# BoxLib-Codes/VARDEN

Measured on AMD Instinct MI355X. Metric: cells*steps/sec on advance_timestep, higher is better.
Workload: dtype f64; 1 GPU; 3D 256x256x256 single-level variable-density bubble, 1 box(es) of 256^3, MAC+HG projection each step (BASELINE.json configs[1]); parallelism=single GPU, cells=16777216

## Files before the change

### varden_amd/csrc/mg_cc.hip

```cpp
#include "vdn_dev.h"
#include "mg_stop.h"
#include "krylov_wg.h"
#include "krylov_grid.h"
#include <chrono>
#include <tuple>
#include <algorithm>

struct CLev {
  int n[3]; int PX, PY; long sz;
  double hi2[3];
  double *phi, *rh, *res, *b[3];
  double *alpha;
  const double *rho;
  int fold[3][2];
  double cmu;
};
DEVI long cidx(const CLev &L, int i, int j, int k) { return (long)(i + 16) + (long)L.PX * ((long)(j + 1) + (long)L.PY * (long)(k + 1)); }

DEVI double beta_of(double ra, double rb, bool at_face, int e) {
  double v = 2.0 / (ra + rb);
  if (at_face) { if (e == VDN_BC_NEU) v = 0.0; else if (e == VDN_BC_DIR) v = 2.0 * v; }
  return v;
}
template <bool RHO = false> DEVI void cc_apply(const CLev &L, long c, double &Ap, double &diag, int i = 0, int j = 0, int k = 0) {
  const long sy = L.PX, sz = (long)L.PX * L.PY;
  const double p0 = L.phi[c];
// ... 652 lines not shown
  DEVI void fill_point(double *v, int t) const { CLev Lv = L; Lv.phi = v; cc_periodic_point(Lv, per, t); }
  KRY_HD long size() const { return L.sz; }
  DEVI const double *rhs() const { return L.rh; }
  DEVI double *x() const { return L.phi; }
  KRY_HD bool singular() const { return sing != 0; }
};
using CcKrylov = CcKrylovT<false>;
using CcKrylovRef = CcKrylovT<true>;
template <bool KRYLOV> __global__ void __launch_bounds__(1024) kk_cc_tailcycle(CcTailArgs T, KrylovTail<KRYLOV> Q) {
  #pragma unroll
  for (int l = 0; l < CC_TAIL_MAX - 1; l++)
    if (l < T.nlev - 1) { wg_cc_gsrb(T.L[l], T.nu1, T.per); wg_cc_down(T.L[l], T.L[l + 1], T.per); }
  #pragma unroll
  for (int l = 0; l < CC_TAIL_MAX; l++)
    if (l == T.nlev - 1) {
      if constexpr (KRYLOV) wg_krylov_any(Q.method, CcKrylovRef{ T.L[l], T.per, Q.singular }, Q.K);
      else wg_cc_gsrb(T.L[l], T.nbot, T.per);
    }
  #pragma unroll
  for (int l = CC_TAIL_MAX - 2; l >= 0; l--)
    if (l < T.nlev - 1) { wg_cc_up(T.L[l], T.L[l + 1]); wg_cc_gsrb(T.L[l], T.nu2, T.per); }
}

constexpr int LT = 8;
constexpr int LW = LT + 8;
struct LdsCell { double b[6], rh, a0; };
template <bool ALPHA> DEVI void lds_load_cell(const CLev &L, long c, LdsCell &q) {
  const long sy = L.PX, sz = (long)L.PX * L.PY;
  q.b[0] = L.b[0][c]; q.b[1] = L.b[0][c + 1]; q.b[2] = L.b[1][c]; q.b[3] = L.b[1][c + sy]; q.b[4] = L.b[2][c]; q.b[5] = L.b[2][c + sz];
  q.rh = L.rh[c]; q.a0 = ALPHA ? L.alpha[c] : 0.0;
}
template <bool ALPHA, int SX, int SP> DEVI void lds_pass(const CLev &L, double *s, const LdsCell (&q)[4], const bool (&inside)[4], int at, int x, int y, int z0, int par0, int color, int reach) {
  const bool xy_ok = x >= 4 - reach && x < 4 + LT + reach && y >= 4 - reach && y < 4 + LT + reach;
  #pragma unroll
  for (int m = 0; m < 4; m++) {
    const int z = z0 + m;
    if (!(xy_ok && inside[m] && z >= 4 - reach && z < 4 + LT + reach && ((par0 + m + color) & 1) == 0)) continue;
    const int a = at + m * SP;
    const double p[7] = { s[a], s[a - 1], s[a + 1], s[a - SX], s[a + SX], s[a - SP], s[a + SP] };
    double Ap, diag; cc_apply_vals(L, p, q[m].b, q[m].a0, ALPHA, Ap, diag);
    if (diag != 0.0) s[a] = p[0] + (q[m].rh - Ap) / diag;
  }
}
template <bool ALPHA> __global__ void __launch_bounds__(1024) kk_cc_lds_down(CLev L, CLev C) {
  constexpr int SX = LW + 2, SP = SX * SX;
  __shared__ double s[SX * SX * SX];
// ... 560 lines not shown
}

static void cc_periodic_t(const CCMG &M, const CLev &L) {
  if (!(M.per[0] || M.per[1] || M.per[2])) return;
  int m = std::max(L.n[0], std::max(L.n[1], L.n[2]));
  hipLaunchKernelGGL(kk_cc_periodic, g3(m, m, 6, BLK), BLK, 0, ctx().stream, L, M.per[0], M.per[1], M.per[2]);
}
static void cc_gsrb_t(const CCMG &M, const CLev &L, int nsweeps) {
  if ((long)L.n[0] * L.n[1] * L.n[2] <= SMALL_LEVEL_CELLS) {
    hipLaunchKernelGGL(kk_cc_bottom, dim3(1), dim3(1024), 0, ctx().stream, L, nsweeps, M.per[0], M.per[1], M.per[2]);
    return;
  }
  for (int s = 0; s < nsweeps; s++) for (int color = 0; color < 2; color++) {
    cc_periodic_t(M, L);
    launch_gsrb(L, color, ctx().stream);
  }
}
static void cc_bottom_t(const CCMG &M, const CLev &L) {
  if (M.kry.w) { mg_krylov_visit(M.kry, 0, ctx().prm.mg_bottom_solver_eps, M.krylov(L)); return; }
  const int N = std::max(L.n[0], std::max(L.n[1], L.n[2]));
  const int ns = std::max(ctx().prm.mg_nub, N * N);
  hipLaunchKernelGGL(kk_cc_bottom, dim3(1), dim3(1024), 0, ctx().stream, L, ns, M.per[0], M.per[1], M.per[2]);
}
static bool cc_small_end(const CCMG &M, int dl, int tl) {
  if (!sw().mg_tailcycle) return false;
  static const long tail_cells = SMALL_LEVEL_CELLS;
  const vdn_params &P = ctx().prm;
  CcTailArgs T; memset(&T, 0, sizeof T);
  int nl = 0;
  if (dl >= 0) {
    if (!M.tail.empty() && !(ctx().nranks == 1 && M.dlev.back().single_box)) return false;
    for (int m = dl; m < (int)M.dlev.size(); m++) {
      const CDLev &D = M.dlev[m];
      if (!(D.single_box && D.boxes.size() == 1 && !D.boxes[0].L.rho && (long)D.ng[0] * D.ng[1] * D.ng[2] <= tail_cells) || nl == CC_TAIL_MAX) return false;
      T.L[nl++] = D.boxes[0].L;
    }
  }
  for (int m = tl; m < (int)M.tail.size(); m++) {
    const CLev &L = M.tail[m];
    if ((long)L.n[0] * L.n[1] * L.n[2] > tail_cells || nl == CC_TAIL_MAX) return false;
    T.L[nl++] = L;
  }
  if (nl < 2) return false;
  const CLev &B = T.L[nl - 1];
  const int N = std::max(B.n[0], std::max(B.n[1], B.n[2]));
  T.nlev = nl; T.nu1 = P.mg_nu1; T.nu2 = P.mg_nu2; T.nbot = std::max(P.mg_nub, N * N);
  for (int d = 0; d < 3; d++) T.per[d] = M.per[d];
  if (M.kry.w) hipLaunchKernelGGL(kk_cc_tailcycle<true>, dim3(1), dim3(1024), 0, ctx().stream, T, KrylovTailArgs{ mg_krylov_args(M.kry, 0, P.mg_bottom_solver_eps), M.kry.method, M.kry_singular });
  else hipLaunchKernelGGL(kk_cc_tailcycle<false>, dim3(1), dim3(1024), 0, ctx().stream, T, NoKrylovTailArgs{});
  return true;
}
static bool cc_lds_tail_level(const CCMG &M, int l) {
  const vdn_params &P = ctx().prm;
  if (!sw().mg_lds || l + 1 >= (int)M.tail.size() || P.mg_nu1 != 2 || P.mg_nu2 != 2 || M.per[0] || M.per[1] || M.per[2]) return false;
  const CLev &L = M.tail[l], &C = M.tail[l + 1];
  if (L.rho) return false;
  for (int d = 0; d < 3; d++) if (L.n[d] % LT || L.n[d] < 2 * LT || L.n[d] > 64 || C.n[d] * 2 != L.n[d]) return false;
  return true;
}
static void cc_vcycle_t(const CCMG &M, int l) {
  const vdn_params &P = ctx().prm;
  if (cc_small_end(M, -1, l)) return;
  const CLev &L = M.tail[l];
  if (l == (int)M.tail.size() - 1) { cc_bottom_t(M, L); return; }
  const CLev &C = M.tail[l + 1];
  if (cc_lds_tail_level(M, l)) {
    const dim3 g((unsigned)(L.n[0] / LT), (unsigned)(L.n[1] / LT), (unsigned)(L.n[2] / LT));
    if (L.alpha) hipLaunchKernelGGL(kk_cc_lds_down<true>, g, dim3(1024), 0, ctx().stream, L, C);
    else hipLaunchKernelGGL(kk_cc_lds_down<false>, g, dim3(1024), 0, ctx().stream, L, C);
    cc_vcycle_t(M, l + 1);
    if (L.alpha) hipLaunchKernelGGL(kk_cc_lds_up<true>, g, dim3(1024), 0, ctx().stream, L, C);
    else hipLaunchKernelGGL(kk_cc_lds_up<false>, g, dim3(1024), 0, ctx().stream, L, C);
    return;
  }
// ... 699 lines not shown
```

### varden_amd/csrc/mg_nd.hip

```cpp
#include "vdn_dev.h"
#include "mg_stop.h"
#include "krylov_wg.h"
#include "krylov_grid.h"
#include "nd_lds_plan.h"
#include <tuple>
#include <algorithm>

struct NLev {
  int n[3]; int PX, PY; long sz;
  double f[3];
  double *phi, *tmp, *b, *res, *sig;
  int dirlo[3], dirhi[3];
  int per[3];
};
DEVI long nidx(const NLev &L, int i, int j, int k) { return (long)(i + 16) + (long)L.PX * ((long)(j + 1) + (long)L.PY * (long)(k + 1)); }
DEVI bool nd_is_dir(const NLev &L, int i, int j, int k) {
  return (i == 0 && L.dirlo[0]) || (i == L.n[0] && L.dirhi[0]) || (j == 0 && L.dirlo[1]) || (j == L.n[1] && L.dirhi[1]) ||
         (k == 0 && L.dirlo[2]) || (k == L.n[2] && L.dirhi[2]);
}
DEVI bool nd_is_shell(const NLev &L, int i, int j, int k, int hm) {
  return ((hm & 1) && i == 0) || ((hm & 2) && i == L.n[0]) || ((hm & 4) && j == 0) || ((hm & 8) && j == L.n[1]) ||
         ((hm & 16) && k == 0) || ((hm & 32) && k == L.n[2]);
}

struct NdW { double w0, w1, w2, w3, w4, w5, w6, w7; int iso; };
DEVI NdW nd_weights(const double f[3]) {
  const double fx = f[0], fy = f[1], fz = f[2];
  const double F = fx + fy + fz;
  NdW W;
  W.w0 = 4.0 * F;
  W.w1 = -4.0 * fx + 2.0 * fy + 2.0 * fz;
  W.w2 = 2.0 * fx - 4.0 * fy + 2.0 * fz;
  W.w3 = -2.0 * fx - 2.0 * fy + fz;
  W.w4 = 2.0 * fx + 2.0 * fy - 4.0 * fz;
  W.w5 = -2.0 * fx + fy - 2.0 * fz;
  W.w6 = fx - 2.0 * fy - 2.0 * fz;
  W.w7 = -F;
  W.iso = (W.w1 == 0.0 && W.w2 == 0.0 && W.w4 == 0.0);
  return W;
}
DEVI void nd_stencil(const NdW &W, const double p[3][3][3], const double sg[2][2][2], double &Kp, double &diag) {
  double cz[2][2], cy[2][2], cx[2][2];
  #pragma unroll
  for (int b = 0; b < 2; b++)
    #pragma unroll
    for (int a = 0; a < 2; a++) {
      cz[b][a] = sg[0][b][a] + sg[1][b][a];
      cy[b][a] = sg[b][0][a] + sg[b][1][a];
      cx[b][a] = sg[b][a][0] + sg[b][a][1];
    }
  const double S8 = (cz[0][0] + cz[0][1]) + (cz[1][0] + cz[1][1]);
  const double p0 = p[1][1][1];
  #define D(c, b, a) (p[c][b][a] - p0)
  double A7 = sg[0][0][0] * D(0, 0, 0);
  A7 = fma(sg[0][0][1], D(0, 0, 2), A7); A7 = fma(sg[0][1][0], D(0, 2, 0), A7); A7 = fma(sg[0][1][1], D(0, 2, 2), A7);
  A7 = fma(sg[1][0][0], D(2, 0, 0), A7); A7 = fma(sg[1][0][1], D(2, 0, 2), A7); A7 = fma(sg[1][1][0], D(2, 2, 0), A7); A7 = fma(sg[1][1][1], D(2, 2, 2), A7);
  double A3 = cz[0][0] * D(1, 0, 0); A3 = fma(cz[0][1], D(1, 0, 2), A3); A3 = fma(cz[1][0], D(1, 2, 0), A3); A3 = fma(cz[1][1], D(1, 2, 2), A3);
  double A5 = cy[0][0] * D(0, 1, 0); A5 = fma(cy[0][1], D(0, 1, 2), A5); A5 = fma(cy[1][0], D(2, 1, 0), A5); A5 = fma(cy[1][1], D(2, 1, 2), A5);
  double A6 = cx[0][0] * D(0, 0, 1); A6 = fma(cx[0][1], D(0, 2, 1), A6); A6 = fma(cx[1][0], D(2, 0, 1), A6); A6 = fma(cx[1][1], D(2, 2, 1), A6);
  const double dg = W.w0 * S8;
  double acc = W.w3 * A3;
  acc = fma(W.w5, A5, acc); acc = fma(W.w6, A6, acc); acc = fma(W.w7, A7, acc);
  if (!W.iso) {
    double A1 = (cz[0][0] + cz[1][0]) * D(1, 1, 0); A1 = fma(cz[0][1] + cz[1][1], D(1, 1, 2), A1);
    double A2 = (cz[0][0] + cz[0][1]) * D(1, 0, 1); A2 = fma(cz[1][0] + cz[1][1], D(1, 2, 1), A2);
    double A4 = (cy[0][0] + cy[0][1]) * D(0, 1, 1); A4 = fma(cy[1][0] + cy[1][1], D(2, 1, 1), A4);
    acc = fma(W.w1, A1, acc); acc = fma(W.w2, A2, acc); acc = fma(W.w4, A4, acc);
  }
  #undef D
  Kp = acc; diag = dg;
}
DEVI void nd_apply(const NLev &L, const double *__restrict__ phi, int i, int j, int k, double &Kp, double &diag) {
  const NdW W = nd_weights(L.f);
  const long sy = L.PX, sz = (long)L.PX * L.PY;
  const long c0 = nidx(L, i, j, k);
  double p[3][3][3], sg[2][2][2];
  #pragma unroll
  for (int c = 0; c < 3; c++)
    #pragma unroll
    for (int b = 0; b < 3; b++)
      #pragma unroll
      for (int a = 0; a < 3; a++) p[c][b][a] = phi[c0 + (a - 1) + (b - 1) * sy + (c - 1) * sz];
  #pragma unroll
  for (int c = 0; c < 2; c++)
    #pragma unroll
    for (int b = 0; b < 2; b++)
      #pragma unroll
      for (int a = 0; a < 2; a++) sg[c][b][a] = L.sig[c0 + (a - 1) + (b - 1) * sy + (c - 1) * sz];
  nd_stencil(W, p, sg, Kp, diag);
}

#define NODE_IJK(L)                                                    \
  const int i = blockIdx.x * blockDim.x + threadIdx.x;                 \
// ... 389 lines not shown
  const int k = (int)blockIdx.z - 1;
  if (i > L.n[0] || j > L.n[1] || k > L.n[2]) return;
  int q[3] = { i, j, k }, s[3] = { i, j, k }; bool g = false, zero = false;
  #pragma unroll
  for (int d = 0; d < 3; d++) {
    if (q[d] < 0) { g = true; if (L.per[d]) s[d] = q[d] + L.n[d]; else zero = true; }
    else if (q[d] >= L.n[d]) { g = true; if (L.per[d]) s[d] = q[d] - L.n[d]; else zero = true; }
  }
  if (g) a[nidx(L, i, j, k)] = zero ? 0.0 : a[nidx(L, s[0], s[1], s[2])];
}
__global__ void kk_nd_restrict(NLev F, NLev C) {
  NODE_IJK(C)
  if (!in_range) return;
  double s = 0.0;
  if (!nd_is_dir(C, i, j, k)) {
    const long sy = F.PX, sz = (long)F.PX * F.PY;
    const long f0 = nidx(F, 2 * i, 2 * j, 2 * k);
    s = nd_fw27(F.res + f0, sy, sz);
  }
  const long cn = nidx(C, i, j, k);
  C.b[cn] = s * 0.125;
  C.phi[cn] = 0.0;
}
DEVI double nd_interp8(const NLev &C, const double *__restrict__ cp, int I, int J, int K, int oi, int oj, int ok) {
  const long c0 = nidx(C, I, J, K), sy = C.PX, sz = (long)C.PX * C.PY;
  const double v000 = cp[c0], v100 = cp[c0 + 1], v010 = cp[c0 + sy], v110 = cp[c0 + sy + 1];
  const double v001 = cp[c0 + sz], v101 = cp[c0 + sz + 1], v011 = cp[c0 + sz + sy], v111 = cp[c0 + sz + sy + 1];
  double s = 0.0;
  s = s + v000;
  s = oi ? s + v100 : s;
  s = oj ? s + v010 : s;
  s = (oi && oj) ? s + v110 : s;
  s = ok ? s + v001 : s;
  s = (ok && oi) ? s + v101 : s;
  s = (ok && oj) ? s + v011 : s;
  s = (ok && oi && oj) ? s + v111 : s;
  return s * (1.0 / (double)((1 + oi) * (1 + oj) * (1 + ok)));
}
__global__ void __launch_bounds__(256) kk_nd_prolong_m(NLev F, NLev C, int c00, int c01, int c02, int kchunk) {
  const int i = blockIdx.x * 64 + threadIdx.x, j = blockIdx.y * 4 + threadIdx.y;
  const int k0 = (int)blockIdx.z * kchunk, k1 = min(k0 + kchunk - 1, F.n[2]);
  if (i > F.n[0] || j > F.n[1] || k0 > k1) return;
  const int oi = i & 1, oj = j & 1;
  const long sy = C.PX, sz = (long)C.PX * C.PY;
  const double *__restrict__ cp = C.phi;
  long c0 = nidx(C, c00 + (i >> 1), c01 + (j >> 1), c02 + (k0 >> 1));
  double a00 = cp[c0], a10 = cp[c0 + 1], a01 = cp[c0 + sy], a11 = cp[c0 + sy + 1];
  const bool dir_ij = (i == 0 && F.dirlo[0]) || (i == F.n[0] && F.dirhi[0]) || (j == 0 && F.dirlo[1]) || (j == F.n[1] && F.dirhi[1]);
  const double w0 = 1.0 / (double)((1 + oi) * (1 + oj)), w1 = 1.0 / (double)((1 + oi) * (1 + oj) * 2);
  for (int k = k0; k <= k1; k += 2) {
    const double b00 = cp[c0 + sz], b10 = cp[c0 + sz + 1], b01 = cp[c0 + sz + sy], b11 = cp[c0 + sz + sy + 1];
    const long f = nidx(F, i, j, k);
    const double pe = F.phi[f];
    const bool odd_in = k + 1 <= k1;
    const long f2 = f + (long)F.PX * F.PY;
    const double po = odd_in ? F.phi[f2] : 0.0;
    double s = 0.0;
    s = s + a00;
    s = oi ? s + a10 : s;
    s = oj ? s + a01 : s;
// ... 297 lines not shown
  KRY_HD long size() const { return L.sz; }
  DEVI const double *rhs() const { return L.b; }
  DEVI double *x() const { return phi; }
  KRY_HD bool singular() const { return !(L.dirlo[0] || L.dirlo[1] || L.dirlo[2] || L.dirhi[0] || L.dirhi[1] || L.dirhi[2]); }
};
using NdKrylov = NdKrylovT<false>;
using NdKrylovRef = NdKrylovT<true>;
template <bool KRYLOV> __global__ void __launch_bounds__(1024) kk_nd_tailcycle(NdTailArgs T, KrylovTail<KRYLOV> Q) {
  double *ph[ND_TAIL_MAX], *tm[ND_TAIL_MAX];
  #pragma unroll
  for (int l = 0; l < ND_TAIL_MAX; l++) { ph[l] = T.L[l].phi; tm[l] = T.L[l].tmp; }
  #pragma unroll
  for (int l = 0; l < ND_TAIL_MAX - 1; l++)
    if (l < T.nlev - 1) { wg_nd_jacobi(T.L[l], ph[l], tm[l], T.nu1, T.omega, T.om1, T.om2, T.nsp); wg_nd_down(T.L[l], ph[l], T.L[l + 1], ph[l + 1]); }
  #pragma unroll
  for (int l = 0; l < ND_TAIL_MAX; l++)
    if (l == T.nlev - 1) {
      if constexpr (KRYLOV) wg_krylov_any(Q.method, NdKrylovRef{ T.L[l], ph[l] }, Q.K);
      else wg_nd_jacobi(T.L[l], ph[l], tm[l], T.nbot, T.omega);
    }
  #pragma unroll
  for (int l = ND_TAIL_MAX - 2; l >= 0; l--)
    if (l < T.nlev - 1) { wg_nd_up(T.L[l], ph[l], T.L[l + 1], ph[l + 1]); wg_nd_jacobi(T.L[l], ph[l], tm[l], T.nu2, T.omega); }
}

__global__ void kk_nd_load_sigma(NLev L, FV coeffs, int lo0, int lo1, int lo2) {
  const int i = (int)(blockIdx.x * blockDim.x + threadIdx.x) - 1;
  const int j = (int)(blockIdx.y * blockDim.y + threadIdx.y) - 1;
  const int k = (int)blockIdx.z - 1;
  if (i > L.n[0] || j > L.n[1] || k > L.n[2]) return;
  L.sig[nidx(L, i, j, k)] = fv_get(coeffs, lo0 + i, lo1 + j, lo2 + k);
}
DEVI void nd_divu_node(const FV &u, const FV &rh, double fx, double fy, double fz, int i, int j, int k) {
  #define U(a, b, c, m) fv_get(u, i + (a), j + (b), k + (c), m)
  const double dux = (((U(0, 0, 0, 0) + U(0, -1, 0, 0)) + U(0, 0, -1, 0)) + U(0, -1, -1, 0))
                   - (((U(-1, 0, 0, 0) + U(-1, -1, 0, 0)) + U(-1, 0, -1, 0)) + U(-1, -1, -1, 0));
  const double duy = (((U(0, 0, 0, 1) + U(-1, 0, 0, 1)) + U(0, 0, -1, 1)) + U(-1, 0, -1, 1))
                   - (((U(0, -1, 0, 1) + U(-1, -1, 0, 1)) + U(0, -1, -1, 1)) + U(-1, -1, -1, 1));
  const double duz = (((U(0, 0, 0, 2) + U(-1, 0, 0, 2)) + U(0, -1, 0, 2)) + U(-1, -1, 0, 2))
                   - (((U(0, 0, -1, 2) + U(-1, 0, -1, 2)) + U(0, -1, -1, 2)) + U(-1, -1, -1, 2));
  #undef U
  fv_at(rh, i, j, k) = fv_get(rh, i, j, k) + (dux * fx + duy * fy + duz * fz);
}
struct nd_divu_K { FV u; FV rh; double fx; double fy; double fz;
  __device__ void cell(int i, int j, int k) const {
    nd_divu_node(u, rh, fx, fy, fz, i, j, k);
// ... 457 lines not shown
static bool nd_prolong_fusable(const NDMG &M, int l) {
  const NDLev &DL = M.dlev[l];
  if (!(sw().nd_prolong_fused && DL.single_box && DL.boxes.size() == 1 && !DL.halo_A && !DL.halo_B && !(DL.per[0] || DL.per[1] || DL.per[2]))) return false;
  if (l + 1 < (int)M.dlev.size() ? M.dlev[l + 1].boxes.size() != 1 : M.tail.empty()) return false;
  const NBox &B = DL.boxes[0];
  const NLev &L = B.L, &C = l + 1 < (int)M.dlev.size() ? M.dlev[l + 1].boxes[0].L : M.tail[0];
  for (int d = 0; d < 3; d++) if (B.lo[d] != 0 || C.n[d] != L.n[d] / 2) return false;
  return nd_wide_even_level(L);
}
static unsigned g_nd_pro_levels = 0;
unsigned nd_last_prolong_levels() { return g_nd_pro_levels; }
static void nd_prolong_smooth(NDMG &M, int l) {
  const int nu2 = ctx().prm.hg_nu2;
  if (nu2 < 1 || !nd_prolong_fusable(M, l)) { nd_prolong_up(M, l); nd_jacobi_d(M.dlev[l], nu2); return; }
  if (l + 1 < (int)M.dlev.size()) nd_halo_phi(M.dlev[l + 1]); else nd_fill_nodes(M.tail[0], M.tail[0].phi);
  const NLev C = l + 1 < (int)M.dlev.size() ? M.dlev[l + 1].boxes[0].L : M.tail[0];
  M.pro_levels |= 1u << l;
  nd_jacobi_d(M.dlev[l], nu2, false, &C);
}
static int nd_bottom_sweeps_global(const NDLev &DL) {
  const int N = std::max(DL.ng[0], std::max(DL.ng[1], DL.ng[2]));
  return std::max(ctx().prm.hg_nub, 2 * N * N);
}
static bool nd_small_end(NDMG &M, int dl, int tl) {
  if (!sw().mg_tailcycle) return false;
  static const long tail_nodes = SMALL_LEVEL_NODES;
  const vdn_params &P = ctx().prm;
  NdTailArgs T; memset(&T, 0, sizeof T);
  int nl = 0;
  if (dl >= 0) {
    if (!M.tail.empty() && !(ctx().nranks == 1 && M.dlev.back().single_box)) return false;
    for (int m = dl; m < (int)M.dlev.size(); m++) {
      const NDLev &D = M.dlev[m];
      if (!(D.single_box && D.boxes.size() == 1 && (long)(D.ng[0] + 1) * (D.ng[1] + 1) * (D.ng[2] + 1) <= tail_nodes) || nl == ND_TAIL_MAX) return false;
      T.L[nl] = D.boxes[0].L; for (int d = 0; d < 3; d++) T.L[nl].per[d] = D.per[d];
      nl++;
    }
  }
  for (int m = tl; m < (int)M.tail.size(); m++) {
    const NLev &L = M.tail[m];
    if ((long)(L.n[0] + 1) * (L.n[1] + 1) * (L.n[2] + 1) > tail_nodes || nl == ND_TAIL_MAX) return false;
    T.L[nl++] = L;
  }
  if (nl < 2) return false;
  const NLev &B = T.L[nl - 1];
  const int N = std::max(B.n[0], std::max(B.n[1], B.n[2]));
  T.nlev = nl; T.nu1 = P.hg_nu1; T.nu2 = P.hg_nu2; T.nbot = std::max(P.hg_nub, 2 * N * N); T.omega = P.hg_omega; { const NdOm o = nd_om(true, P.hg_nu1); T.om1 = o.om1; T.om2 = o.om2; T.nsp = o.nsp; }
  if (M.kry.w) { hipLaunchKernelGGL(kk_nd_tailcycle<true>, dim3(1), dim3(1024), 0, ctx().stream, T, KrylovTailArgs{ mg_krylov_args(M.kry, 1, P.hg_bottom_solver_eps), M.kry.method, 0 }); T.nbot = 0;  }
  else hipLaunchKernelGGL(kk_nd_tailcycle<false>, dim3(1), dim3(1024), 0, ctx().stream, T, NoKrylovTailArgs{});
  int m = 0;
  if (dl >= 0) for (int q = dl; q < (int)M.dlev.size(); q++, m++) {
    const int sweeps = (m == nl - 1) ? T.nbot : T.nu1 + T.nu2;
    if (sweeps & 1) { NDLev &D = M.dlev[q]; std::swap(D.boxes[0].L.phi, D.boxes[0].L.tmp); D.flip = !D.flip; }
  }
  for (int q = tl; q < (int)M.tail.size(); q++, m++) {
    const int sweeps = (m == nl - 1) ? T.nbot : T.nu1 + T.nu2;
    if (sweeps & 1) std::swap(M.tail[q].phi, M.tail[q].tmp);
  }
  return true;
}
static bool nd_lds_level(const NDMG &M, int l) {
  const vdn_params &P = ctx().prm;
  if (!sw().mg_lds || l < 1 || l + 1 >= (int)M.dlev.size() || ctx().nranks != 1 || P.hg_nu1 != 2 || P.hg_nu2 != 1 || M.per[0] || M.per[1] || M.per[2]) return false;
  const NDLev &D = M.dlev[l], &DC = M.dlev[l + 1];
  if (!(D.single_box && D.boxes.size() == 1 && !D.halo_A && !D.halo_B && !D.halo_res && !(D.per[0] || D.per[1] || D.per[2]) && DC.single_box && DC.boxes.size() == 1)) return false;
  const NBox &B = D.boxes[0];
  for (int d = 0; d < 3; d++) if (!nd_lds_extent_ok(B.L.n[d]) || B.lo[d] != 0 || DC.boxes[0].L.n[d] * 2 != B.L.n[d]) return false;
  return true;
}
static unsigned g_nd_lds_levels = 0;
unsigned nd_last_lds_levels() { return g_nd_lds_levels; }
static void nd_vcycle_d(NDMG &M, int l) {
// ... 1093 lines not shown
```

### varden_amd/csrc/runtime.hip

```cpp
#include "vdn_dev.h"
#include <algorithm>
#include <chrono>
#include <map>
#include <tuple>

static VdnCtx g_ctx;
VdnCtx &ctx() { return g_ctx; }
static thread_local char g_err[1024] = "";

void vdn_set_error(const char *fmt, ...) { va_list ap; va_start(ap, fmt); vsnprintf(g_err, sizeof g_err, fmt, ap); va_end(ap); }
void vdn_fail(const char *fmt, ...) {
  char buf[1024]; va_list ap; va_start(ap, fmt); vsnprintf(buf, sizeof buf, fmt, ap); va_end(ap);
  throw VdnErr(buf);
}

static std::vector<vdn_multifab *> g_temp_mfs;
void arena_reset() {
  dbg_sync(16);
  for (vdn_multifab *m : g_temp_mfs) delete m;
  g_temp_mfs.clear();
  if (sw().arena_poison && g_ctx.arena && g_ctx.arena_peak > 0) HIPCHK(hipMemsetAsync(g_ctx.arena, 0xFF, std::min(g_ctx.arena_peak + (size_t)(64 << 20), g_ctx.arena_bytes), g_ctx.stream));
  g_ctx.arena_off = 0;
  g_ctx.drop_step_caches();
}
// ... 141 lines not shown
extern char **environ;
static void env_warn_unknown() {
  static bool done = false;
  if (done) return;
  done = true;
  for (char **e = environ; e && *e; e++) {
    if (strncmp(*e, "VDN_", 4) != 0 || !strncmp(*e, "VDN_BENCH_", 10) || !strncmp(*e, "VDN_WORKER_", 11)) continue;
    const char *eq = strchr(*e, '=');
    const size_t len = eq ? (size_t)(eq - *e) : strlen(*e);
    bool known = false;
    for (const SwitchInfo &s : switch_table) if (strlen(s.name) == len && !strncmp(s.name, *e, len)) known = true;
    if (!strncmp(*e, "VDN_LIB_FLAVOUR", 15)) continue;
    if (!known) fprintf(stderr, "varden_amd: warning: environment variable %.*s is not a switch of this library (vdn_debug_switches lists them)\n", (int)len, *e);
#ifndef VDN_TESTING_BUILD
    else fprintf(stderr, "varden_amd: note: %.*s is set but this is the release build: launch-form switches are compiled out (libvarden_amd_testing.so reads them)\n", (int)len, *e);
#endif
  }
}
#ifdef VDN_TESTING_BUILD
unsigned nd_last_prolong_levels();
extern "C" unsigned vdn_nd_prolong_fused_levels(void) { return nd_last_prolong_levels(); }
unsigned nd_last_lds_levels();
extern "C" unsigned vdn_nd_lds_levels(void) { return nd_last_lds_levels(); }
#endif
extern "C" const char *vdn_debug_switches(void) {
  static std::string out;
#ifndef VDN_TESTING_BUILD
  if (out.empty()) out = "release build: the switches below are compiled out, every launch form is the default one (libvarden_amd_testing.so reads them)\n";
#endif
  if (out.find(std::string(switch_table[0].name) + " ") == std::string::npos) for (const SwitchInfo &s : switch_table) { const char *v = switch_raw(s); out += s.name; out += v ? std::string(" = ") + v : std::string(" (unset)"); out += ": "; out += s.doc; out += "\n"; }
  return out.c_str();
}

bool g_capturing_now();
__global__ void k_publish(double *host_view, const double *dev, int n, unsigned long long seq) {
  if ((int)threadIdx.x < n) host_view[threadIdx.x] = dev[threadIdx.x];
  __syncthreads();
  if (threadIdx.x == 0) { __threadfence_system(); *reinterpret_cast<volatile unsigned long long *>(host_view + 64) = seq; }
}
const double *read_scalars(const double *dev, int n) {
  VdnCtx &c = g_ctx;
  REQUIRE(n >= 1 && n <= 64, "read_scalars: 1..64 values");
  static unsigned long long seq = 0;
  const bool poll = sw().poll >= 0 ? sw().poll != 0 : c.nranks == 1;
  ++seq;
  dbg_sync(8);
// ... 750 lines not shown
```

Before: 688.1 million cells*steps/s.

## Run small multigrid tail V-cycles entirely in LDS for cell and node solvers

```diff
diff --git a/varden_amd/csrc/mg_cc.hip b/varden_amd/csrc/mg_cc.hip
--- a/varden_amd/csrc/mg_cc.hip
+++ b/varden_amd/csrc/mg_cc.hip
@@ -2,6 +2,7 @@
 #include "mg_stop.h"
 #include "krylov_wg.h"
 #include "krylov_grid.h"
+#include "tail_plan.h"
 #include <chrono>
 #include <tuple>
 #include <algorithm>
@@ -700,6 +701,115 @@
     if (l < T.nlev - 1) { wg_cc_up(T.L[l], T.L[l + 1]); wg_cc_gsrb(T.L[l], T.nu2, T.per); }
 }
 
+struct CcTailLdsArgs { CLev L[TAIL_MAX_LEVELS]; TailPlan P; int nu1, nu2, nbot, per[3]; };
+struct CcOwn {
+  double b[6], a0, rh, diag, res;
+  long gc;
+  int lc, rc, up;
+  int fine;
+  int colour, img;
+  bool ok;
+};
+DEVI void cct_enter(const CcTailLdsArgs &T, int l, CcOwn &o) {
+  const CLev &L = T.L[l]; const TailLevel &P = T.P.L[l];
+  int i, j, k;
+  o.ok = tail_owner(TAIL_CELLS, P.n, threadIdx.x, i, j, k, o.colour);
+  o.gc = cidx(L, i, j, k);
+  o.lc = P.phi + tail_index(P, i, j, k);
+  o.rc = T.P.res + i + P.n[0] * (j + P.n[1] * k);
+  o.up = l + 1 < T.P.nlev ? T.P.L[l + 1].phi + tail_index(T.P.L[l + 1], i >> 1, j >> 1, k >> 1) : 0;
+  o.fine = l > 0 ? T.P.res + 2 * i + T.P.L[l - 1].n[0] * (2 * j + T.P.L[l - 1].n[1] * 2 * k) : 0;
+  o.img = 0;
+  const int q[3] = { i, j, k };
+  for (int d = 0; d < 3; d++) if (T.per[d]) { if (q[d] == 0) o.img |= 1 << (2 * d); if (q[d] == P.n[d] - 1) o.img |= 2 << (2 * d); }
+  const long sy = L.PX, sz = (long)L.PX * L.PY;
+  for (int m = 0; m < 6; m++) o.b[m] = 0.0;
+  o.a0 = 0.0; o.rh = 0.0; o.res = 0.0;
+  if (o.ok) {
+    o.b[0] = L.b[0][o.gc]; o.b[1] = L.b[0][o.gc + 1];
+    o.b[2] = L.b[1][o.gc]; o.b[3] = L.b[1][o.gc + sy];
+    o.b[4] = L.b[2][o.gc]; o.b[5] = L.b[2][o.gc + sz];
+    if (L.alpha) o.a0 = L.alpha[o.gc];
+    if (l == 0) o.rh = L.rh[o.gc];
+  }
+  const double p[7] = { 0.0, 0.0, 0.0, 0.0, 0.0, 0.0, 0.0 };
+  double Ap; cc_apply_vals(L, p, o.b, o.a0, L.alpha != nullptr, Ap, o.diag);
+}
+DEVI double cct_apply(const CLev &L, const TailLevel &P, const double *lds, const CcOwn &o, double &p0) {
+  const int sy = P.e[0], sz = P.e[0] * P.e[1];
+  const double p[7] = { lds[o.lc], lds[o.lc - 1], lds[o.lc + 1], lds[o.lc - sy], lds[o.lc + sy], lds[o.lc - sz], lds[o.lc + sz] };
+  double Ap, diag; cc_apply_vals(L, p, o.b, o.a0, L.alpha != nullptr, Ap, diag);
+  p0 = p[0];
+  return Ap;
+}
+DEVI void cct_put(const TailLevel &P, double *lds, const CcOwn &o, double v) {
+  lds[o.lc] = v;
+  if (o.img) {
+    const int st[3] = { 1, P.e[0], P.e[0] * P.e[1] };
+    #pragma unroll
+    for (int d = 0; d < 3; d++) {
+      if (o.img & (1 << (2 * d))) lds[o.lc + P.n[d] * st[d]] = v;
+      if (o.img & (2 << (2 * d))) lds[o.lc - P.n[d] * st[d]] = v;
+    }
+  }
+}
+DEVI void cct_gsrb(const CLev &L, const TailLevel &P, double *lds, const CcOwn &o, int nsweeps) {
+  for (int s = 0; s < nsweeps; s++) for (int color = 0; color < 2; color++) {
+    if (o.ok && o.colour == color) {
+      double p0; const double Ap = cct_apply(L, P, lds, o, p0);
+      if (o.diag != 0.0) cct_put(P, lds, o, p0 + (o.rh - Ap) / o.diag);
+    }
+    __syncthreads();
+  }
+}
+__global__ void __launch_bounds__(TAIL_THREADS) kk_cc_tailcycle_lds(CcTailLdsArgs T) {
+  __shared__ double lds[TAIL_LDS_DOUBLES];
+  CcOwn o[TAIL_MAX_LEVELS];
+  #pragma unroll
+  for (int l = 0; l < TAIL_MAX_LEVELS; l++) if (l < T.P.nlev) cct_enter(T, l, o[l]);
+  {
+    const CLev &L = T.L[0]; const TailLevel &P = T.P.L[0];
+    for (int t = threadIdx.x; t < tail_array(P); t += TAIL_THREADS) {
+      int q[3] = { t % P.e[0] - 1, (t / P.e[0]) % P.e[1] - 1, t / (P.e[0] * P.e[1]) - 1 };
+      for (int d = 0; d < 3; d++) if (T.per[d]) { if (q[d] < 0) q[d] += P.n[d]; else if (q[d] >= P.n[d]) q[d] -= P.n[d]; }
+      lds[P.phi + t] = L.phi[cidx(L, q[0], q[1], q[2])];
+    }
+  }
+  __syncthreads();
+  #pragma unroll
+  for (int l = 0; l < TAIL_MAX_LEVELS - 1; l++)
+    if (l < T.P.nlev - 1) {
+      const CLev &L = T.L[l]; const TailLevel &P = T.P.L[l], &PC = T.P.L[l + 1];
+      cct_gsrb(L, P, lds, o[l], T.nu1);
+      if (o[l].ok) { double p0; o[l].res = o[l].rh - cct_apply(L, P, lds, o[l], p0); lds[o[l].rc] = o[l].res; }
+      for (int t = threadIdx.x; t < tail_array(PC); t += TAIL_THREADS) lds[PC.phi + t] = 0.0;
+      __syncthreads();
+      if (o[l + 1].ok) {
+        const double *r = lds; const int f = o[l + 1].fine, sy = P.n[0], sz = P.n[0] * P.n[1];
+        const double s = r[f] + r[f + 1] + r[f + sy] + r[f + sy + 1] + r[f + sz] + r[f + sz + 1] + r[f + sz + sy] + r[f + sz + sy + 1];
+        o[l + 1].rh = s * 0.125;
+      }
+      if (T.nu1 == 0) __syncthreads();
+    }
+  #pragma unroll
+  for (int l = 0; l < TAIL_MAX_LEVELS; l++)
+    if (l == T.P.nlev - 1) cct_gsrb(T.L[l], T.P.L[l], lds, o[l], T.nbot);
+  #pragma unroll
+  for (int l = TAIL_MAX_LEVELS - 2; l >= 0; l--)
+    if (l < T.P.nlev - 1) {
+      if (o[l].ok) cct_put(T.P.L[l], lds, o[l], lds[o[l].lc] + lds[o[l].up]);
+      __syncthreads();
+      cct_gsrb(T.L[l], T.P.L[l], lds, o[l], T.nu2);
+    }
+  #pragma unroll
+  for (int l = 0; l < TAIL_MAX_LEVELS; l++)
+    if (l < T.P.nlev && o[l].ok) {
+      T.L[l].phi[o[l].gc] = lds[o[l].lc];
+      if (l > 0) T.L[l].rh[o[l].gc] = o[l].rh;
+      if (l < T.P.nlev - 1) T.L[l].res[o[l].gc] = o[l].res;
+    }
+}
+
 constexpr int LT = 8;
 constexpr int LW = LT + 8;
 struct LdsCell { double b[6], rh, a0; };
@@ -1306,7 +1416,9 @@
   const int ns = std::max(ctx().prm.mg_nub, N * N);
   hipLaunchKernelGGL(kk_cc_bottom, dim3(1), dim3(1024), 0, ctx().stream, L, ns, M.per[0], M.per[1], M.per[2]);
 }
+static int g_cc_tail_form = 0;
 static bool cc_small_end(const CCMG &M, int dl, int tl) {
+  g_cc_tail_form = 0;
   if (!sw().mg_tailcycle) return false;
   static const long tail_cells = SMALL_LEVEL_CELLS;
   const vdn_params &P = ctx().prm;
@@ -1330,10 +1442,24 @@
   const int N = std::max(B.n[0], std::max(B.n[1], B.n[2]));
   T.nlev = nl; T.nu1 = P.mg_nu1; T.nu2 = P.mg_nu2; T.nbot = std::max(P.mg_nub, N * N);
   for (int d = 0; d < 3; d++) T.per[d] = M.per[d];
-  if (M.kry.w) hipLaunchKernelGGL(kk_cc_tailcycle<true>, dim3(1), dim3(1024), 0, ctx().stream, T, KrylovTailArgs{ mg_krylov_args(M.kry, 0, P.mg_bottom_solver_eps), M.kry.method, M.kry_singular });
-  else hipLaunchKernelGGL(kk_cc_tailcycle<false>, dim3(1), dim3(1024), 0, ctx().stream, T, NoKrylovTailArgs{});
+  g_cc_tail_form = 0;
+  if (M.kry.w) { hipLaunchKernelGGL(kk_cc_tailcycle<true>, dim3(1), dim3(1024), 0, ctx().stream, T, KrylovTailArgs{ mg_krylov_args(M.kry, 0, P.mg_bottom_solver_eps), M.kry.method, M.kry_singular }); return true; }
+  int tn[TAIL_MAX_LEVELS][3] = {};
+  for (int l = 0; l < std::min(nl, TAIL_MAX_LEVELS); l++) for (int d = 0; d < 3; d++) tn[l][d] = T.L[l].n[d];
+  const TailPlan TP = tail_plan(TAIL_CELLS, nl, tn, T.per);
+  if (TP.fits) {
+    CcTailLdsArgs A; memset(&A, 0, sizeof A);
+    for (int l = 0; l < nl; l++) A.L[l] = T.L[l];
+    A.P = TP; A.nu1 = T.nu1; A.nu2 = T.nu2; A.nbot = T.nbot;
+    for (int d = 0; d < 3; d++) A.per[d] = T.per[d];
+    hipLaunchKernelGGL(kk_cc_tailcycle_lds, dim3(1), dim3(TAIL_THREADS), 0, ctx().stream, A);
+    g_cc_tail_form = 1;
+    return true;
+  }
+  hipLaunchKernelGGL(kk_cc_tailcycle<false>, dim3(1), dim3(1024), 0, ctx().stream, T, NoKrylovTailArgs{});
   return true;
 }
+int cc_last_tail_form() { return g_cc_tail_form; }
 static bool cc_lds_tail_level(const CCMG &M, int l) {
   const vdn_params &P = ctx().prm;
   if (!sw().mg_lds || l + 1 >= (int)M.tail.size() || P.mg_nu1 != 2 || P.mg_nu2 != 2 || M.per[0] || M.per[1] || M.per[2]) return false;
diff --git a/varden_amd/csrc/mg_nd.hip b/varden_amd/csrc/mg_nd.hip
--- a/varden_amd/csrc/mg_nd.hip
+++ b/varden_amd/csrc/mg_nd.hip
@@ -3,6 +3,7 @@
 #include "krylov_wg.h"
 #include "krylov_grid.h"
 #include "nd_lds_plan.h"
+#include "tail_plan.h"
 #include <tuple>
 #include <algorithm>
 
@@ -39,17 +40,22 @@
   W.iso = (W.w1 == 0.0 && W.w2 == 0.0 && W.w4 == 0.0);
   return W;
 }
-DEVI void nd_stencil(const NdW &W, const double p[3][3][3], const double sg[2][2][2], double &Kp, double &diag) {
-  double cz[2][2], cy[2][2], cx[2][2];
+struct NdCoef { double sg[2][2][2], cz[2][2], cy[2][2], cx[2][2], dg; };
+DEVI void nd_stencil_coef(const NdW &W, const double sg[2][2][2], NdCoef &K) {
   #pragma unroll
   for (int b = 0; b < 2; b++)
     #pragma unroll
     for (int a = 0; a < 2; a++) {
-      cz[b][a] = sg[0][b][a] + sg[1][b][a];
-      cy[b][a] = sg[b][0][a] + sg[b][1][a];
-      cx[b][a] = sg[b][a][0] + sg[b][a][1];
-    }
-  const double S8 = (cz[0][0] + cz[0][1]) + (cz[1][0] + cz[1][1]);
+      K.sg[0][b][a] = sg[0][b][a]; K.sg[1][b][a] = sg[1][b][a];
+      K.cz[b][a] = sg[0][b][a] + sg[1][b][a];
+      K.cy[b][a] = sg[b][0][a] + sg[b][1][a];
+      K.cx[b][a] = sg[b][a][0] + sg[b][a][1];
+    }
+  const double S8 = (K.cz[0][0] + K.cz[0][1]) + (K.cz[1][0] + K.cz[1][1]);
+  K.dg = W.w0 * S8;
+}
+DEVI void nd_stencil_apply(const NdW &W, const double p[3][3][3], const NdCoef &K, double &Kp) {
+  const auto &sg = K.sg; const auto &cz = K.cz; const auto &cy = K.cy; const auto &cx = K.cx;
   const double p0 = p[1][1][1];
   #define D(c, b, a) (p[c][b][a] - p0)
   double A7 = sg[0][0][0] * D(0, 0, 0);
@@ -58,7 +64,6 @@
   double A3 = cz[0][0] * D(1, 0, 0); A3 = fma(cz[0][1], D(1, 0, 2), A3); A3 = fma(cz[1][0], D(1, 2, 0), A3); A3 = fma(cz[1][1], D(1, 2, 2), A3);
   double A5 = cy[0][0] * D(0, 1, 0); A5 = fma(cy[0][1], D(0, 1, 2), A5); A5 = fma(cy[1][0], D(2, 1, 0), A5); A5 = fma(cy[1][1], D(2, 1, 2), A5);
   double A6 = cx[0][0] * D(0, 0, 1); A6 = fma(cx[0][1], D(0, 2, 1), A6); A6 = fma(cx[1][0], D(2, 0, 1), A6); A6 = fma(cx[1][1], D(2, 2, 1), A6);
-  const double dg = W.w0 * S8;
   double acc = W.w3 * A3;
   acc = fma(W.w5, A5, acc); acc = fma(W.w6, A6, acc); acc = fma(W.w7, A7, acc);
   if (!W.iso) {
@@ -68,7 +73,13 @@
     acc = fma(W.w1, A1, acc); acc = fma(W.w2, A2, acc); acc = fma(W.w4, A4, acc);
   }
   #undef D
-  Kp = acc; diag = dg;
+  Kp = acc;
+}
+DEVI void nd_stencil(const NdW &W, const double p[3][3][3], const double sg[2][2][2], double &Kp, double &diag) {
+  NdCoef K;
+  nd_stencil_coef(W, sg, K);
+  nd_stencil_apply(W, p, K, Kp);
+  diag = K.dg;
 }
 DEVI void nd_apply(const NLev &L, const double *__restrict__ phi, int i, int j, int k, double &Kp, double &diag) {
   const NdW W = nd_weights(L.f);
@@ -504,8 +515,7 @@
   C.b[cn] = s * 0.125;
   C.phi[cn] = 0.0;
 }
-DEVI double nd_interp8(const NLev &C, const double *__restrict__ cp, int I, int J, int K, int oi, int oj, int ok) {
-  const long c0 = nidx(C, I, J, K), sy = C.PX, sz = (long)C.PX * C.PY;
+DEVI double nd_interp8_at(const double *__restrict__ cp, long c0, long sy, long sz, int oi, int oj, int ok) {
   const double v000 = cp[c0], v100 = cp[c0 + 1], v010 = cp[c0 + sy], v110 = cp[c0 + sy + 1];
   const double v001 = cp[c0 + sz], v101 = cp[c0 + sz + 1], v011 = cp[c0 + sz + sy], v111 = cp[c0 + sz + sy + 1];
   double s = 0.0;
@@ -518,6 +528,9 @@
   s = (ok && oj) ? s + v011 : s;
   s = (ok && oi && oj) ? s + v111 : s;
   return s * (1.0 / (double)((1 + oi) * (1 + oj) * (1 + ok)));
+}
+DEVI double nd_interp8(const NLev &C, const double *__restrict__ cp, int I, int J, int K, int oi, int oj, int ok) {
+  return nd_interp8_at(cp, nidx(C, I, J, K), C.PX, (long)C.PX * C.PY, oi, oj, ok);
 }
 __global__ void __launch_bounds__(256) kk_nd_prolong_m(NLev F, NLev C, int c00, int c01, int c02, int kchunk) {
   const int i = blockIdx.x * 64 + threadIdx.x, j = blockIdx.y * 4 + threadIdx.y;
@@ -861,6 +874,137 @@
   #pragma unroll
   for (int l = ND_TAIL_MAX - 2; l >= 0; l--)
     if (l < T.nlev - 1) { wg_nd_up(T.L[l], ph[l], T.L[l + 1], ph[l + 1]); wg_nd_jacobi(T.L[l], ph[l], tm[l], T.nu2, T.omega); }
+}
+
+struct NdTailLdsArgs { NLev L[TAIL_MAX_LEVELS]; TailPlan P; int nu1, nu2, nbot; double omega, om1, om2; int nsp; };
+struct NdOwn {
+  double b;
+  int ijk;
+  bool ok, dir;
+  DEVI int i() const { return ijk & 1023; }
+  DEVI int j() const { return (ijk >> 10) & 1023; }
+  DEVI int k() const { return ijk >> 20; }
+  DEVI int lc(const TailLevel &P) const { return tail_index(P, i(), j(), k()); }
+  DEVI int sc(const TailLevel &P) const { return i() + (P.n[0] + 2) * (j() + (P.n[1] + 2) * k()); }
+};
+DEVI void ndt_enter(const NdTailLdsArgs &T, int l, NdOwn &o) {
+  const NLev &L = T.L[l]; const TailLevel &P = T.P.L[l];
+  int i, j, k, colour;
+  o.ok = tail_owner(TAIL_NODES, P.n, threadIdx.x, i, j, k, colour);
+  o.dir = nd_is_dir(L, i, j, k);
+  o.ijk = i | (j << 10) | (k << 20);
+  o.b = (l == 0 && o.ok) ? L.b[nidx(L, i, j, k)] : 0.0;
+}
+DEVI void ndt_coef(const NdW &W, const TailLevel &P, const double *lds, const NdOwn &o, NdCoef &K) {
+  const int sy = P.n[0] + 2, sz = (P.n[0] + 2) * (P.n[1] + 2);
+  const double *s = lds + P.sig + o.sc(P);
+  double sg[2][2][2];
+  #pragma unroll
+  for (int c = 0; c < 2; c++)
+    #pragma unroll
+    for (int b = 0; b < 2; b++)
+      #pragma unroll
+      for (int a = 0; a < 2; a++) sg[c][b][a] = s[a + b * sy + c * sz];
+  nd_stencil_coef(W, sg, K);
+}
+DEVI double ndt_apply(const NdW &W, const TailLevel &P, const double *src, int lc, const NdCoef &K, double &p0) {
+  const int sy = P.e[0], sz = P.e[0] * P.e[1];
+  double p[3][3][3];
+  #pragma unroll
+  for (int c = 0; c < 3; c++)
+    #pragma unroll
+    for (int b = 0; b < 3; b++)
+      #pragma unroll
+      for (int a = 0; a < 3; a++) p[c][b][a] = src[lc + (a - 1) + (b - 1) * sy + (c - 1) * sz];
+  double Kp; nd_stencil_apply(W, p, K, Kp);
+  p0 = p[1][1][1];
+  return Kp;
+}
+DEVI void ndt_jacobi(const NdW &W, const TailLevel &P, double *lds, const NdOwn &o, const NdCoef &K, int &cur, int nsweeps, double omega, double om1 = 0.0, double om2 = 0.0, int nsp = 0) {
+  const int lc = o.lc(P);
+  for (int s = 0; s < nsweeps; s++) {
+    const double *src = lds + (cur ? P.tmp : P.phi);
+    double *dst = lds + (cur ? P.phi : P.tmp);
+    if (o.ok) {
+      double p0 = src[lc], v = p0;
+      if (!o.dir) {
+        const double Kp = ndt_apply(W, P, src, lc, K, p0);
+        v = p0;
+        if (K.dg != 0.0) v = p0 + (s < nsp ? (s == 0 ? om1 : om2) : omega) * ((o.b - Kp) / K.dg);
+      }
+      dst[lc] = v;
+    }
+    __syncthreads();
+    cur ^= 1;
+  }
+}
+__global__ void __launch_bounds__(TAIL_THREADS) kk_nd_tailcycle_lds(NdTailLdsArgs T) {
+  __shared__ double lds[TAIL_LDS_DOUBLES];
+  NdOwn o[TAIL_MAX_LEVELS];
+  int cur[TAIL_MAX_LEVELS];
+  #pragma unroll
+  for (int l = 0; l < TAIL_MAX_LEVELS; l++) { cur[l] = 0; if (l < T.P.nlev) ndt_enter(T, l, o[l]); }
+  for (int t = threadIdx.x; t < T.P.total; t += TAIL_THREADS) lds[t] = 0.0;
+  __syncthreads();
+  #pragma unroll
+  for (int l = 0; l < TAIL_MAX_LEVELS; l++)
+    if (l < T.P.nlev) {
+      const NLev &L = T.L[l]; const TailLevel &P = T.P.L[l];
+      const int s0 = P.n[0] + 2, s1 = P.n[1] + 2, ns = s0 * s1 * (P.n[2] + 2);
+      for (int t = threadIdx.x; t < ns; t += TAIL_THREADS) lds[P.sig + t] = L.sig[nidx(L, t % s0 - 1, (t / s0) % s1 - 1, t / (s0 * s1) - 1)];
+      if (l == 0) for (int t = threadIdx.x; t < tail_array(P); t += TAIL_THREADS) lds[P.phi + t] = L.phi[nidx(L, t % P.e[0] - 1, (t / P.e[0]) % P.e[1] - 1, t / (P.e[0] * P.e[1]) - 1)];
+    }
+  __syncthreads();
+  #pragma unroll
+  for (int l = 0; l < TAIL_MAX_LEVELS - 1; l++)
+    if (l < T.P.nlev - 1) {
+      const TailLevel &P = T.P.L[l];
+      const NdW W = nd_weights(T.L[l].f);
+      NdCoef K; ndt_coef(W, P, lds, o[l], K);
+      ndt_jacobi(W, P, lds, o[l], K, cur[l], T.nu1, T.omega, T.om1, T.om2, T.nsp);
+      if (o[l].ok) {
+        double r = 0.0;
+        if (!o[l].dir) { double p0; r = o[l].b - ndt_apply(W, P, lds + (cur[l] ? P.tmp : P.phi), o[l].lc(P), K, p0); }
+        lds[P.res + o[l].lc(P)] = r;
+      }
+      __syncthreads();
+      if (o[l + 1].ok) {
+        double s = 0.0;
+        if (!o[l + 1].dir) s = nd_fw27(lds + P.res + tail_index(P, 2 * o[l + 1].i(), 2 * o[l + 1].j(), 2 * o[l + 1].k()), P.e[0], P.e[0] * P.e[1]);
+        o[l + 1].b = s * 0.125;
+      }
+    }
+  #pragma unroll
+  for (int l = 0; l < TAIL_MAX_LEVELS; l++)
+    if (l == T.P.nlev - 1) {
+      const NdW W = nd_weights(T.L[l].f);
+      NdCoef K; ndt_coef(W, T.P.L[l], lds, o[l], K);
+      ndt_jacobi(W, T.P.L[l], lds, o[l], K, cur[l], T.nbot, T.omega);
+    }
+  #pragma unroll
+  for (int l = TAIL_MAX_LEVELS - 2; l >= 0; l--)
+    if (l < T.P.nlev - 1) {
+      const TailLevel &P = T.P.L[l], &PC = T.P.L[l + 1];
+      double *fphi = lds + (cur[l] ? P.tmp : P.phi);
+      if (o[l].ok && !o[l].dir) {
+        const int i = o[l].i(), j = o[l].j(), k = o[l].k(), lc = o[l].lc(P);
+        fphi[lc] = fphi[lc] + nd_interp8_at(lds + (cur[l + 1] ? PC.tmp : PC.phi), tail_index(PC, i >> 1, j >> 1, k >> 1), PC.e[0], PC.e[0] * PC.e[1], i & 1, j & 1, k & 1);
+      }
+      __syncthreads();
+      const NdW W = nd_weights(T.L[l].f);
+      NdCoef K; ndt_coef(W, P, lds, o[l], K);
+      ndt_jacobi(W, P, lds, o[l], K, cur[l], T.nu2, T.omega);
+    }
+  #pragma unroll
+  for (int l = 0; l < TAIL_MAX_LEVELS; l++)
+    if (l < T.P.nlev && o[l].ok) {
+      const TailLevel &P = T.P.L[l];
+      const long gc = nidx(T.L[l], o[l].i(), o[l].j(), o[l].k());
+      const int lc = o[l].lc(P);
+      (cur[l] ? T.L[l].tmp : T.L[l].phi)[gc] = lds[(cur[l] ? P.tmp : P.phi) + lc];
+      if (l > 0) T.L[l].b[gc] = o[l].b;
+      if (l < T.P.nlev - 1) T.L[l].res[gc] = lds[P.res + lc];
+    }
 }
 
 __global__ void kk_nd_load_sigma(NLev L, FV coeffs, int lo0, int lo1, int lo2) {
@@ -1364,7 +1508,10 @@
   const int N = std::max(DL.ng[0], std::max(DL.ng[1], DL.ng[2]));
   return std::max(ctx().prm.hg_nub, 2 * N * N);
 }
+static int g_nd_tail_form = 0;
+int nd_last_tail_form() { return g_nd_tail_form; }
 static bool nd_small_end(NDMG &M, int dl, int tl) {
+  g_nd_tail_form = 0;
   if (!sw().mg_tailcycle) return false;
   static const long tail_nodes = SMALL_LEVEL_NODES;
   const vdn_params &P = ctx().prm;
@@ -1389,7 +1536,18 @@
   const int N = std::max(B.n[0], std::max(B.n[1], B.n[2]));
   T.nlev = nl; T.nu1 = P.hg_nu1; T.nu2 = P.hg_nu2; T.nbot = std::max(P.hg_nub, 2 * N * N); T.omega = P.hg_omega; { const NdOm o = nd_om(true, P.hg_nu1); T.om1 = o.om1; T.om2 = o.om2; T.nsp = o.nsp; }
   if (M.kry.w) { hipLaunchKernelGGL(kk_nd_tailcycle<true>, dim3(1), dim3(1024), 0, ctx().stream, T, KrylovTailArgs{ mg_krylov_args(M.kry, 1, P.hg_bottom_solver_eps), M.kry.method, 0 }); T.nbot = 0;  }
-  else hipLaunchKernelGGL(kk_nd_tailcycle<false>, dim3(1), dim3(1024), 0, ctx().stream, T, NoKrylovTailArgs{});
+  else {
+    int tn[TAIL_MAX_LEVELS][3] = {}, per[3] = { 0, 0, 0 };
+    for (int l = 0; l < nl; l++) for (int d = 0; d < 3; d++) { if (l < TAIL_MAX_LEVELS) tn[l][d] = T.L[l].n[d]; if (T.L[l].per[d]) per[d] = 1; }
+    const TailPlan TP = tail_plan(TAIL_NODES, nl, tn, per);
+    if (TP.fits) {
+      NdTailLdsArgs A; memset(&A, 0, sizeof A);
+      for (int l = 0; l < nl; l++) A.L[l] = T.L[l];
+      A.P = TP; A.nu1 = T.nu1; A.nu2 = T.nu2; A.nbot = T.nbot; A.omega = T.omega; A.om1 = T.om1; A.om2 = T.om2; A.nsp = T.nsp;
+      hipLaunchKernelGGL(kk_nd_tailcycle_lds, dim3(1), dim3(TAIL_THREADS), 0, ctx().stream, A);
+      g_nd_tail_form = 1;
+    } else hipLaunchKernelGGL(kk_nd_tailcycle<false>, dim3(1), dim3(1024), 0, ctx().stream, T, NoKrylovTailArgs{});
+  }
   int m = 0;
   if (dl >= 0) for (int q = dl; q < (int)M.dlev.size(); q++, m++) {
     const int sweeps = (m == nl - 1) ? T.nbot : T.nu1 + T.nu2;
diff --git a/varden_amd/csrc/runtime.hip b/varden_amd/csrc/runtime.hip
--- a/varden_amd/csrc/runtime.hip
+++ b/varden_amd/csrc/runtime.hip
@@ -187,6 +187,9 @@
 extern "C" unsigned vdn_nd_prolong_fused_levels(void) { return nd_last_prolong_levels(); }
 unsigned nd_last_lds_levels();
 extern "C" unsigned vdn_nd_lds_levels(void) { return nd_last_lds_levels(); }
+int cc_last_tail_form();
+int nd_last_tail_form();
+extern "C" int vdn_last_tail_form(int which) { return which == 0 ? cc_last_tail_form() : nd_last_tail_form(); }
 #endif
 extern "C" const char *vdn_debug_switches(void) {
   static std::string out;
diff --git a/varden_amd/csrc/tail_plan.h b/varden_amd/csrc/tail_plan.h
--- /dev/null
+++ b/varden_amd/csrc/tail_plan.h
@@ -0,0 +1,74 @@
+#pragma once
+#if defined(__HIPCC__)
+#define TAIL_FN __host__ __device__ inline
+#else
+#define TAIL_FN inline
+#endif
+
+#define TAIL_THREADS 1024
+#define TAIL_MAX_LEVELS 3
+#define TAIL_LDS_DOUBLES 7680
+#define TAIL_CELLS 0
+#define TAIL_NODES 1
+
+struct TailLevel {
+  int n[3];
+  int e[3];
+  int phi, tmp, res, sig;
+};
+struct TailPlan {
+  int kind, nlev, fits;
+  TailLevel L[TAIL_MAX_LEVELS];
+  int res;
+  int total;
+};
+
+TAIL_FN int tail_points(int kind, const int n[3]) { return kind == TAIL_CELLS ? n[0] * n[1] * n[2] : (n[0] + 1) * (n[1] + 1) * (n[2] + 1); }
+TAIL_FN int tail_threads(int kind, const int n[3]) { return kind == TAIL_CELLS ? 2 * ((n[0] + 1) / 2) * n[1] * n[2] : tail_points(kind, n); }
+TAIL_FN bool tail_owner(int kind, const int n[3], int t, int &i, int &j, int &k, int &colour) {
+  i = j = k = colour = 0;
+  if (t < 0 || t >= tail_threads(kind, n)) return false;
+  if (kind == TAIL_CELLS) {
+    const int half = (n[0] + 1) / 2, th = half * n[1] * n[2];
+    colour = t / th;
+    const int q = t - colour * th;
+    k = q / (half * n[1]); j = (q / half) % n[1];
+    i = 2 * (q % half) + ((j + k + colour) & 1);
+    if (i >= n[0]) { i = 0; return false; }
+    return true;
+  }
+  const int m0 = n[0] + 1, m1 = n[1] + 1;
+  i = t % m0; j = (t / m0) % m1; k = t / (m0 * m1);
+  return true;
+}
+TAIL_FN int tail_index(const TailLevel &L, int i, int j, int k) { return (i + 1) + L.e[0] * ((j + 1) + L.e[1] * (k + 1)); }
+TAIL_FN int tail_array(const TailLevel &L) { return L.e[0] * L.e[1] * L.e[2]; }
+
+TAIL_FN TailPlan tail_plan(int kind, int nlev, const int (*n)[3], const int per[3]) {
+  TailPlan P;
+  P.kind = kind; P.nlev = nlev; P.fits = 0; P.res = 0; P.total = 0;
+  for (int l = 0; l < TAIL_MAX_LEVELS; l++) for (int d = 0; d < 3; d++) { P.L[l].n[d] = P.L[l].e[d] = 0; P.L[l].phi = P.L[l].tmp = P.L[l].res = P.L[l].sig = 0; }
+  if (nlev < 2 || nlev > TAIL_MAX_LEVELS) return P;
+  const int g = kind == TAIL_CELLS ? 2 : 3;
+  long off = 0;
+  bool ok = true;
+  for (int l = 0; l < nlev; l++) {
+    TailLevel &L = P.L[l];
+    long arr = 1;
+    for (int d = 0; d < 3; d++) {
+      if (n[l][d] < 1 || n[l][d] > TAIL_THREADS) return P;
+      L.n[d] = n[l][d]; L.e[d] = n[l][d] + g; arr *= L.e[d];
+      if (l > 0 && 2 * n[l][d] != n[l - 1][d]) ok = false;
+      if (per[d] && (kind == TAIL_NODES || (n[l][d] & 1))) ok = false;
+    }
+    if ((long)L.n[0] * L.n[1] * L.n[2] > TAIL_THREADS || tail_threads(kind, L.n) > TAIL_THREADS) return P;
+    L.phi = (int)off; off += arr;
+    if (kind == TAIL_NODES) { L.tmp = (int)off; off += arr; L.res = (int)off; off += arr; L.sig = (int)off; off += (long)(L.n[0] + 2) * (L.n[1] + 2) * (L.n[2] + 2); }
+    if (off > TAIL_LDS_DOUBLES) return P;
+  }
+  if (kind == TAIL_CELLS) { P.res = (int)off; off += (long)n[0][0] * n[0][1] * n[0][2]; }
+  P.total = (int)off;
+  P.fits = ok && off <= TAIL_LDS_DOUBLES;
+  return P;
+}
+TAIL_FN long tail_lds_bytes(const TailPlan &P) { return 8L * P.total; }
```

New measurement: 702.7 million cells*steps/s, median of 6. 1.02x the previous value.
